# MaverickPeter/MR_SLAM

Hardware: AMD Instinct MI355X
Metric: loop-candidate pairs/sec (BEV+Radon+corr), 120k-pt scans (higher is better)
Workload: dtype f32; 1 GPU; BASELINE configs[1] batched: 120k-pt synthetic lidar scans -> Cartesian BEV 120x120x1 -> Radon 120x120 -> normalise -> half spectrum -> FFT-domain rotation correlation vs 1 candidate of the database (+ 1 query per launch swept over the database)

## Files before the change

mr_slam_amd/csrc/ringfft.hip:

```cpp
#include <algorithm>
#include <atomic>
#include <cmath>
#include <cstdlib>
#include <type_traits>

#include <hip/hip_fp16.h>

#include "common.hpp"
#include "fft_codelets.hpp"

namespace {

constexpr int kA = 120;
constexpr int kD = 120;
constexpr int kHalf = 61;
constexpr int kSlotThreads = 128;

constexpr int kLdsStride = 128;

__device__ __forceinline__ v2f cmul_conj(v2f a, v2f b)
{
    const v2f t = a.yx * b.yy * (v2f){1.0f, -1.0f};
    return __builtin_elementwise_fma(a, b.xx, t);
}

__device__ __forceinline__ v2f twiddle120(int K, v2f d)
{
    const v2f t = d.yx * (v2f){-kSin120[K], kSin120[K]};
    return __builtin_elementwise_fma(d, (v2f){kCos120[K], kCos120[K]}, t);
}

__device__ __forceinline__ void irfft_pre_pair(int J, v2f u, v2f w, v2f& zj, v2f& zp)
{
    const v2f e = __builtin_elementwise_fma(w, (v2f){1.0f, -1.0f}, u);
    const v2f d = __builtin_elementwise_fma(w, (v2f){-1.0f, 1.0f}, u);
    const v2f o = twiddle120(J, d);
    zj = __builtin_elementwise_fma(o.yx, (v2f){-1.0f, 1.0f}, e);
    zp = __builtin_elementwise_fma(e, (v2f){1.0f, -1.0f}, o.yx);
}

constexpr int kPairsPerGroup = 5;
template <class LoadA, class LoadB>
__device__ __forceinline__ void corr_irfft120(LoadA la, LoadB lb, v2f (&x)[60])
{
    constexpr int G = kPairsPerGroup, NG = 30 / kPairsPerGroup;
    v2f abuf[2][2 * G + 1];
    auto request = [&](int g, v2f (&dst)[2 * G + 1]) {
#pragma unroll
        for (int j = 0; j < G; ++j) {
            dst[2 * j] = la(g * G + j);
            dst[2 * j + 1] = la(60 - (g * G + j));
        }
        if (g == NG - 1) dst[2 * G] = la(30);
    };
    request(0, abuf[0]);
#pragma unroll
    for (int g = 0; g < NG; ++g) {
        if (g + 1 < NG) request(g + 1, abuf[(g + 1) & 1]);
        __builtin_amdgcn_sched_barrier(0);
        const v2f(&a)[2 * G + 1] = abuf[g & 1];
#pragma unroll
        for (int j = 0; j < G; ++j) {
            const int J = g * G + j;
            v2f zj, zp;
            irfft_pre_pair(J, cmul_conj(a[2 * j], lb(J)), cmul_conj(a[2 * j + 1], lb(60 - J)), zj, zp);
            x[J] = zj;
            if (J != 0) x[60 - J] = zp;
        }
        if (g == NG - 1) {
            const v2f pm = cmul_conj(a[2 * G], lb(30));
            v2f unused;
            irfft_pre_pair(30, pm, pm, x[30], unused);
        }
    }
    cfft60_inv(x);
}

__device__ __forceinline__ void rfft_post_pair(int K, v2f zk, v2f zp, v2f& xk, v2f& xp)
{
    const v2f sum = __builtin_elementwise_fma(zp, (v2f){1.0f, -1.0f}, zk);
    const v2f d = __builtin_elementwise_fma(zp, (v2f){-1.0f, 1.0f}, zk);
    const v2f tt = d.yx * (v2f){kSin120[K], -kSin120[K]};
    const v2f t = __builtin_elementwise_fma(d, (v2f){kCos120[K], kCos120[K]}, tt);
    xk = __builtin_elementwise_fma(t.yx, (v2f){1.0f, -1.0f}, sum);
    xp = __builtin_elementwise_fma(sum, (v2f){1.0f, -1.0f}, -t.yx);
}

template <class Store>
__device__ __forceinline__ void rfft120(v2f (&x)[60], Store store)
{
    cfft60_fwd(x);
#pragma unroll
    for (int K = 0; K <= 30; ++K) {
        v2f xk, xp;
        rfft_post_pair(K, x[K], x[(60 - K) % 60], xk, xp);
        store(K, xk);
        if (K != 30) store(60 - K, xp);
    }
}

constexpr float kOrtho120 = 0.09128709291752769f;

__global__ __launch_bounds__(kSlotThreads) void k_ring_half_spectrum(const float* __restrict__ x, float2* __restrict__ out,
                                                                     __half2* __restrict__ out16)
{
    const int d = min((int)threadIdx.x, kD - 1);
    const float* src = x + (size_t)blockIdx.x * kA * kD + d;
    v2f s[60];
#pragma unroll
    for (int m = 0; m < 60; ++m) s[m] = (v2f){src[(2 * m) * kD], src[(2 * m + 1) * kD]};
    const bool live = threadIdx.x < kD;
    const size_t o = (size_t)blockIdx.x * kHalf * kD + d;
    rfft120(s, [&](int k, v2f twice) {
        if (!live) return;
        const v2f v = twice * (v2f){0.5f * kOrtho120, 0.5f * kOrtho120};
        if (out) out[o + k * kD] = make_float2(v.x, v.y);
        if (out16) out16[o + k * kD] = __floats2half2_rn(v.x, v.y);
    });
}

__device__ __forceinline__ float swap32_abs_add(float a, float b)
{
    const auto r = __builtin_amdgcn_permlane32_swap(__float_as_uint(a), __float_as_uint(b), false, false);
    return fabsf(__uint_as_float(r[0])) + fabsf(__uint_as_float(r[1]));
}
__device__ __forceinline__ float swap16_add(float a, float b)
{
    const auto r = __builtin_amdgcn_permlane16_swap(__float_as_uint(a), __float_as_uint(b), false, false);
    return __uint_as_float(r[0]) + __uint_as_float(r[1]);
}

__device__ __forceinline__ void wave_abs_reduce_scatter(const v2f (&x)[60], float& w0, float& w1)
{
    const int lane = threadIdx.x & 63;
    float w[64];
#pragma unroll
    for (int i = 0; i < 64; ++i) {
        const int j = 64 + i;
        const float lo_v = (i & 1) ? x[i >> 1].y : x[i >> 1].x;
        const float hi_v = j < 120 ? ((j & 1) ? x[j >> 1].y : x[j >> 1].x) : 0.0f;
        w[i] = swap32_abs_add(lo_v, hi_v);
    }
#pragma unroll
    for (int i = 0; i < 32; ++i) w[i] = swap16_add(w[i], w[32 + i]);
#pragma unroll
    for (int step = 2; step < 6; ++step) {
        const int keep = 64 >> step;
        const int mask = 32 >> step;
        const bool hi = (lane & mask) != 0;
#pragma unroll
        for (int i = 0; i < keep; ++i) {
            const float send = hi ? w[i] : w[keep + i];
            const float mine = hi ? w[keep + i] : w[i];
            w[i] = mine + __shfl_xor(send, mask, 64);
        }
    }
    w0 = w[0];
    w1 = w[1];
}

struct FftCorrP {
    int nq, ndb, pairwise, channels;
    float denom;
    const long long* db_first;
    const long long* q_row;
    float2* mc_partial;
    int units;
};

__device__ __forceinline__ float2 load_spec(const float2* p) { return *p; }
__device__ __forceinline__ float2 load_spec(const __half2* p) { return __half22float2(*p); }

template <int NSLOT, bool QLDS, bool PAIRWISE, bool MULTI, typename DBT, bool PRELOAD = false>
__global__ __launch_bounds__(NSLOT* kSlotThreads) void k_ring_corr_fft(const float2* __restrict__ Q, const DBT* __restrict__ DB,
                                                                       FftCorrP p, float* __restrict__ dist,
                                                                       int* __restrict__ angle, float* __restrict__ corr_out)
{
    extern __shared__ __attribute__((aligned(16))) v2f qs[];
    __shared__ float xbuf[NSLOT][128];
    const int q = blockIdx.y;
    const int slot = threadIdx.x / kSlotThreads;
    const int t = threadIdx.x % kSlotThreads;
    const int wave_in_slot = t >> 6, lane = t & 63;
    const int d = min(t, kD - 1);
    const bool live_col = t < kD;
    const int C = MULTI ? p.channels : 1;
    const size_t entry = (size_t)C * kHalf * kD;
    const float2* qsrc = Q + (size_t)((!PAIRWISE && p.q_row) ? p.q_row[q] : q) * entry;
    if (!PAIRWISE && p.db_first) DB += (size_t)p.db_first[q] * entry;
    if (QLDS) {
        for (int i = threadIdx.x; i < kHalf * kLdsStride; i += NSLOT * kSlotThreads) {
            const int k = i / kLdsStride, col = i % kLdsStride;
            v2f v = {0.0f, 0.0f};
            if (col < kD) { const float2 g = qsrc[k * kD + col]; v = (v2f){g.x, g.y}; }
            qs[i] = v;
        }
        __syncthreads();
    }
    const int ncand = PAIRWISE ? 1 : p.ndb;
    const int stride = gridDim.x * NSLOT;
    const int rounds = (ncand + stride - 1) / stride;
    for (int r = 0; r < rounds; ++r) {
        const int cand = (r * gridDim.x + blockIdx.x) * NSLOT + slot;
        const bool live = cand < ncand;
        float v[2] = {0.0f, 0.0f};
        if (live) {
            for (int c = 0; c < C; ++c) {
                v2f x[60];
                const DBT* b = DB + (size_t)(PAIRWISE ? q : cand) * entry + (size_t)c * kHalf * kD + d;
                const float2* a = qsrc + (size_t)c * kHalf * kD + d;
                auto la = [&](int k) {
                    if (QLDS) return qs[k * kLdsStride + t];
                    const float2 g = a[k * kD];
                    return live_col ? (v2f){g.x, g.y} : (v2f){0.0f, 0.0f};
                };
                if (PRELOAD) {
                    DBT raw[kHalf];
#pragma unroll
                    for (int k = 0; k < kHalf; ++k) raw[k] = b[k * kD];
                    __builtin_amdgcn_sched_barrier(0);
                    corr_irfft120(la, [&](int k) { const float2 g = load_spec(&raw[k]); return (v2f){g.x, g.y}; }, x);
                } else {
                    corr_irfft120(la, [&](int k) { const float2 g = load_spec(b + k * kD); return (v2f){g.x, g.y}; }, x);
                }
                float w0, w1;
                wave_abs_reduce_scatter(x, w0, w1);
                v[0] += w0;
                v[1] += w1;
            }
        }
        if (wave_in_slot == 1) { xbuf[slot][2 * lane] = v[0]; xbuf[slot][2 * lane + 1] = v[1]; }
        __syncthreads();
        if (wave_in_slot == 0 && live) {
            const float sc = kOrtho120;
            const float s0 = (v[0] + xbuf[slot][2 * lane]) * sc, s1 = (v[1] + xbuf[slot][2 * lane + 1]) * sc;
            const int n0 = 2 * lane, n1 = 2 * lane + 1;
            const int m0 = n0 < 60 ? n0 + 60 : n0 - 60, m1 = n1 < 60 ? n1 + 60 : n1 - 60;
            const size_t o = (size_t)q * (PAIRWISE ? 1 : p.ndb) + (PAIRWISE ? 0 : cand);
            float best = -1.0f;
            int bm = 1 << 30;
            if (lane < 60) {
                if (corr_out) { corr_out[o * kA + m0] = s0; corr_out[o * kA + m1] = s1; }
                best = s0; bm = m0;
                if (s1 > best || (s1 == best && m1 < bm)) { best = s1; bm = m1; }
            }
            for (int off = 32; off > 0; off >>= 1) {
                const float ob = __shfl_xor(best, off, 64);
                const int om = __shfl_xor(bm, off, 64);
                if (ob > best || (ob == best && om < bm)) { best = ob; bm = om; }
            }
            if (lane == 0) {
                dist[o] = 1.0f - best / p.denom;
                angle[o] = kA / 2 - bm;
            }
        }
        __syncthreads();
    }
}

template <int NSLOT, typename DBT, int WAVES>
__global__ __launch_bounds__(NSLOT* kSlotThreads) __attribute__((amdgpu_waves_per_eu(WAVES, WAVES))) void k_ring_sweep_pipe(
    const float2* __restrict__ Q, const DBT* __restrict__ DB, FftCorrP p, float* __restrict__ dist, int* __restrict__ angle,
    float* __restrict__ corr_out)
{
    extern __shared__ __attribute__((aligned(16))) v2f qs[];
    __shared__ float xbuf[NSLOT][128];
    const int q = blockIdx.y;
    const int slot = threadIdx.x / kSlotThreads;
    const int t = threadIdx.x % kSlotThreads;
    const int wave_in_slot = t >> 6, lane = t & 63;
    const int d = min(t, kD - 1);
    const size_t entry = (size_t)kHalf * kD;
    const float2* qsrc = Q + (size_t)q * entry;
    const int ncand = p.ndb;
    const int stride = gridDim.x * NSLOT;
    const int rounds = (ncand + stride - 1) / stride;
    int cand = blockIdx.x * NSLOT + slot;
    DBT nxt[kHalf];
    auto fetch = [&](int c) {
        const DBT* b = DB + (size_t)c * entry + d;
#pragma unroll
        for (int k = 0; k < kHalf; ++k) nxt[k] = b[k * kD];
    };
    if (cand < ncand) fetch(cand);
    for (int i = threadIdx.x; i < kHalf * kLdsStride; i += NSLOT * kSlotThreads) {
        const int k = i / kLdsStride, col = i % kLdsStride;
        v2f v = {0.0f, 0.0f};
        if (col < kD) { const float2 g = qsrc[k * kD + col]; v = (v2f){g.x, g.y}; }
        qs[i] = v;
    }
    __syncthreads();
    for (int r = 0; r < rounds; ++r) {
        const bool live = cand < ncand;
        DBT cur[kHalf];
#pragma unroll
        for (int k = 0; k < kHalf; ++k) cur[k] = nxt[k];
        const int next = cand + stride;
        if (next < ncand) fetch(next);
        __builtin_amdgcn_sched_barrier(0);
        float v0 = 0.0f, v1 = 0.0f;
        if (live) {
            v2f x[60];
            corr_irfft120([&](int k) { return qs[k * kLdsStride + t]; },
                          [&](int k) { const float2 g = load_spec(&cur[k]); return (v2f){g.x, g.y}; }, x);
            wave_abs_reduce_scatter(x, v0, v1);
        }
        if (wave_in_slot == 1) { xbuf[slot][2 * lane] = v0; xbuf[slot][2 * lane + 1] = v1; }
        __syncthreads();
        if (wave_in_slot == 0 && live) {
            const float sc = kOrtho120;
            const float s0 = (v0 + xbuf[slot][2 * lane]) * sc, s1 = (v1 + xbuf[slot][2 * lane + 1]) * sc;
            const int n0 = 2 * lane, n1 = 2 * lane + 1;
            const int m0 = n0 < 60 ? n0 + 60 : n0 - 60, m1 = n1 < 60 ? n1 + 60 : n1 - 60;
            const size_t o = (size_t)q * p.ndb + cand;
            float best = -1.0f;
            int bm = 1 << 30;
            if (lane < 60) {
                if (corr_out) { corr_out[o * kA + m0] = s0; corr_out[o * kA + m1] = s1; }
                best = s0; bm = m0;
                if (s1 > best || (s1 == best && m1 < bm)) { best = s1; bm = m1; }
            }
            for (int off = 32; off > 0; off >>= 1) {
                const float ob = __shfl_xor(best, off, 64);
                const int om = __shfl_xor(bm, off, 64);
                if (ob > best || (ob == best && om < bm)) { best = ob; bm = om; }
            }
            if (lane == 0) {
                dist[o] = 1.0f - best / p.denom;
                angle[o] = kA / 2 - bm;
            }
        }
        __syncthreads();
        cand = next;
    }
}

constexpr int kRing = 8;
constexpr int kElems = 32;
constexpr int kSlotBytes = 1024;
constexpr int kTiledHalf1 = 30 * 1024 + 512;
constexpr int kTiledEntryBytes = 58624;
constexpr int kTiledEntry = kTiledEntryBytes / 8;


#define MRS_GLDS(MOD) asm volatile("s_mov_b32 %0, m0\n\ts_mov_b32 m0, %3\n\ts_nop 0\n\tglobal_load_lds_dwordx4 %1, %2" MOD "\n\ts_mov_b32 m0, %0" \
                                   : "=&s"(keep) : "v"(voff), "s"(sbase), "s"(lds_dst) : "memory")
template <bool NT>
__device__ __forceinline__ void glds16(const void* sbase, unsigned voff, unsigned lds_dst)
{
    unsigned keep;
    if (NT) MRS_GLDS(" nt");
    else MRS_GLDS("");
}
#undef MRS_GLDS

template <int N>
__device__ __forceinline__ void wait_vmcnt()
{
    asm volatile("s_waitcnt vmcnt(%0)" ::"n"(N) : "memory");
}

__device__ __forceinline__ void wave_abs_reduce_scatter_masked(const v2f (&x)[60], float m, float& w0, float& w1)
{
    const int lane = threadIdx.x & 63;
    float w[64];
#pragma unroll
    for (int i = 0; i < 64; ++i) {
        const int j = 64 + i;
        const float lo_v = (i & 1) ? x[i >> 1].y : x[i >> 1].x;
        const float hi_v = j < 120 ? ((j & 1) ? x[j >> 1].y : x[j >> 1].x) : 0.0f;
        const auto r = __builtin_amdgcn_permlane32_swap(__float_as_uint(lo_v), __float_as_uint(hi_v), false, false);
        w[i] = __builtin_fmaf(fabsf(__uint_as_float(r[1])), m, fabsf(__uint_as_float(r[0])));
    }
#pragma unroll
    for (int i = 0; i < 32; ++i) w[i] = swap16_add(w[i], w[32 + i]);
#pragma unroll
    for (int step = 2; step < 6; ++step) {
        const int keep = 64 >> step;
        const int mask = 32 >> step;
        const bool hi = (lane & mask) != 0;
#pragma unroll
        for (int i = 0; i < keep; ++i) {
            const float send = hi ? w[i] : w[keep + i];
            const float mine = hi ? w[keep + i] : w[i];
            w[i] = mine + __shfl_xor(send, mask, 64);
        }
    }
    w0 = w[0];
    w1 = w[1];
}

__device__ __forceinline__ void sweep_epilogue(float s0, float s1, int lane, float denom, float* dist_o, int* angle_o)
{
    const int n0 = 2 * lane, n1 = 2 * lane + 1;
    const int m0 = n0 < 60 ? n0 + 60 : n0 - 60, m1 = n1 < 60 ? n1 + 60 : n1 - 60;
    float best = -1.0f;
    int bm = 1 << 30;
    if (lane < 60) {
        best = s0; bm = m0;
        if (s1 > best || (s1 == best && m1 < bm)) { best = s1; bm = m1; }
    }
    for (int off = 32; off > 0; off >>= 1) {
        const float ob = __shfl_xor(best, off, 64);
        const int om = __shfl_xor(bm, off, 64);
        if (ob > best || (ob == best && om < bm)) { best = ob; bm = om; }
    }
    if (lane == 0) {
        *dist_o = 1.0f - best / denom;
        *angle_o = kA / 2 - bm;
    }
}

struct DmaUnit {
    const float2* base;
    int half;
    bool live;
};

template <int WAVES, bool NT, bool TILED, bool MC>
__global__ __launch_bounds__(WAVES * 64) void k_ring_sweep_dma(const float2* __restrict__ Q, const float2* __restrict__ DB, FftCorrP p,
                                                               float* __restrict__ dist, int* __restrict__ angle)
{
    extern __shared__ __attribute__((aligned(1024))) unsigned char smem[];
    v2f* const qs = reinterpret_cast<v2f*>(smem + WAVES * kRing * kSlotBytes);
    constexpr int kQueryVals = kHalf * kD + 8;
    const int wave = __builtin_amdgcn_readfirstlane(threadIdx.x >> 6);
    const int lane = threadIdx.x & 63;
    const unsigned lds0 = (unsigned)(size_t)(__attribute__((address_space(3))) unsigned char*)smem;
    const unsigned ring_lds = lds0 + wave * (kRing * kSlotBytes);
    const v2f* const ring = reinterpret_cast<const v2f*>(smem + wave * (kRing * kSlotBytes)) + lane;

    const size_t plane = TILED ? (size_t)kTiledEntry : (size_t)kHalf * kD;
    const size_t entry = (MC ? (size_t)p.channels : (size_t)1) * plane;
    const size_t qentry = (size_t)kHalf * kD;
    const int ncand = p.ndb;
    const bool multi = p.units > 0;
    const int bx = multi ? (int)((blockIdx.x >> 3) / p.nq) * 8 + (int)(blockIdx.x & 7) : (int)blockIdx.x;
    const int nbx = multi ? p.units : (int)gridDim.x;
    const int qy = multi ? (int)((blockIdx.x >> 3) % p.nq) : (int)blockIdx.y;
    if (multi && bx >= nbx) return;
    const int C = MC ? p.channels : 1;
    const int ch = MC ? bx % C : 0;
    const int slice = MC ? bx / C : bx;
    const int nslices = MC ? (nbx - ch + C - 1) / C : nbx;
    const int c0 = slice * WAVES + wave;
    const int cstride = nslices * WAVES;
    unsigned* const ticket = reinterpret_cast<unsigned*>(qs + kQueryVals);
    auto cand_of = [&](unsigned t) { return slice * WAVES + (int)(t % WAVES) + (int)(t / WAVES) * cstride; };

    const int piece = lane & 31;
    const bool upper = lane >= 32;
    const unsigned voff_h0 = TILED ? (unsigned)lane * 16u : (upper ? 60u * 960u : 0u) + (unsigned)piece * 16u;
    const unsigned voff_h1 = TILED ? (unsigned)kTiledHalf1 + (upper ? 448u : 0u) + (unsigned)min(piece, 27) * 16u
                                   : (upper ? 60u * 960u : 0u) + 512u + (unsigned)min(piece, 27) * 16u;
    const int vdelta = upper ? -960 : 960;
    unsigned run = 0;
    auto start_unit = [&](const DmaUnit& u) {
        run = u.half ? voff_h1 : voff_h0;
        asm volatile("" : "+v"(run));
    };
    auto issue = [&](const DmaUnit& u, int e) {
        if (e == 0) start_unit(u);
        const unsigned voff = (!u.live || e == kElems - 1) ? 0u : run;
        glds16<NT>(u.base, voff, ring_lds + (e % kRing) * kSlotBytes);
        if (TILED) run += u.half ? 896u : 1024u;
        else run += (unsigned)vdelta;
    };
    auto unit_of = [&](int c, int h) {
        DmaUnit u;
        u.live = c < ncand;
        u.base = DB + (size_t)(u.live ? c : 0) * entry + (size_t)ch * plane;
        u.half = h;
        return u;
    };

    const float2* const qsrc = Q + ((size_t)qy * C + (size_t)ch) * qentry;
    {
        constexpr int kPieces = (kHalf * kD * 8 + kSlotBytes - 1) / kSlotBytes;
        const unsigned q_lds = lds0 + WAVES * (kRing * kSlotBytes);
        if (threadIdx.x < 8) qs[kHalf * kD + threadIdx.x] = (v2f){0.0f, 0.0f};
        for (int pc = wave; pc < kPieces; pc += WAVES)
            if (pc * kSlotBytes + lane * 16 < kHalf * kD * 8) glds16<false>(qsrc, (unsigned)(pc * kSlotBytes + lane * 16), q_lds + pc * kSlotBytes);
    }
    DmaUnit cur = unit_of(c0, 0);
#pragma unroll
    for (int e = 0; e < kRing; ++e) issue(cur, e);
    wait_vmcnt<kRing>();
    if (threadIdx.x == 0) *ticket = WAVES;
    asm volatile("s_waitcnt lgkmcnt(0)\n\ts_barrier" ::: "memory");

    constexpr int PF = 2;
    int c = c0;
    float accA0 = 0.0f, accA1 = 0.0f;
    while (cur.live) {
        DmaUnit nxt;
        int c_next = c + cstride;
        if (cur.half == 0) nxt = unit_of(c, 1);
        else {
            unsigned t = 0;
            if (lane == 0) t = __hip_atomic_fetch_add(ticket, 1u, __ATOMIC_RELAXED, __HIP_MEMORY_SCOPE_WORKGROUP);
            c_next = cand_of(__builtin_amdgcn_readfirstlane(t));
            nxt = unit_of(c_next, 0);
        }
        const int h = cur.half;
        const v2f* const qcol = qs + h * 64 + lane;
        const float m = (h == 1 && piece >= 24) ? 0.0f : 1.0f;

        v2f x[60];
        v2f qa[PF + 1][2], cb[PF + 1][2];
        auto read_elem = [&](int e) {
            const int J = e;
            qa[e % (PF + 1)][0] = qcol[J * kD];
            cb[e % (PF + 1)][0] = ring[(e % kRing) * 128];
            if (e < 30) {
                qa[e % (PF + 1)][1] = qcol[(60 - J) * kD];
                cb[e % (PF + 1)][1] = ring[(e % kRing) * 128 + 64];
            }
        };
        __builtin_amdgcn_s_setprio(1);
        wait_vmcnt<kRing - 1>(); read_elem(0);
        wait_vmcnt<kRing - 2>(); read_elem(1);
#pragma unroll
        for (int e = 0; e < kElems; ++e) {
            if (e + PF <= 30) {
                wait_vmcnt<kRing - 1 - PF>();
                read_elem(e + PF);
            }
            if (e < 30) {
                v2f zj, zp;
                irfft_pre_pair(e, cmul_conj(qa[e % (PF + 1)][0], cb[e % (PF + 1)][0]), cmul_conj(qa[e % (PF + 1)][1], cb[e % (PF + 1)][1]), zj, zp);
                x[e] = zj;
                if (e != 0) x[60 - e] = zp;
            } else if (e == 30) {
                const v2f pm = cmul_conj(qa[e % (PF + 1)][0], cb[e % (PF + 1)][0]);
                v2f unused;
                irfft_pre_pair(30, pm, pm, x[30], unused);
            }
            __builtin_amdgcn_sched_barrier(0);
            if (e + kRing < kElems) issue(cur, e + kRing);
            else issue(nxt, e + kRing - kElems);
        }
        __builtin_amdgcn_s_setprio(0);
        cfft60_inv(x);
        float w0, w1;
        wave_abs_reduce_scatter_masked(x, m, w0, w1);

        if (MC) {
            p.mc_partial[(((size_t)qy * C + ch) * p.ndb + c) * 128 + h * 64 + lane] = make_float2(w0, w1);
            if (h == 1) c = c_next;
        } else if (h == 0) {
            accA0 = w0; accA1 = w1;
        } else {
            const float s0 = (accA0 + w0) * kOrtho120, s1 = (accA1 + w1) * kOrtho120;
            const size_t o = (size_t)qy * p.ndb + c;
            sweep_epilogue(s0, s1, lane, p.denom, dist + o, angle + o);
            c = c_next;
        }
        cur = nxt;
    }
    wait_vmcnt<0>();
}

__global__ __launch_bounds__(256) void k_ring_mc_finish(const float2* __restrict__ partial, int ndb, int C, float denom, float* __restrict__ dist,
                                                        int* __restrict__ angle)
{
    const int cand = blockIdx.x * 4 + (threadIdx.x >> 6), lane = threadIdx.x & 63;
    if (cand >= ndb) return;
    partial += (size_t)blockIdx.y * C * ndb * 128;
    float2 lo = make_float2(0.0f, 0.0f), hi = make_float2(0.0f, 0.0f);
    for (int c = 0; c < C; ++c) {
        const float2 a = partial[((size_t)c * ndb + cand) * 128 + lane], b = partial[((size_t)c * ndb + cand) * 128 + 64 + lane];
        lo.x += a.x; lo.y += a.y; hi.x += b.x; hi.y += b.y;
    }
    const size_t o = (size_t)blockIdx.y * ndb + cand;
    sweep_epilogue((lo.x + hi.x) * kOrtho120, (lo.y + hi.y) * kOrtho120, lane, denom, dist + o, angle + o);
}

__global__ __launch_bounds__(256) void k_ring_spec_to_tiled(const float2* __restrict__ src, float2* __restrict__ dst)
{
    const float2* s = src + (size_t)blockIdx.x * kHalf * kD;
    float2* d = dst + (size_t)blockIdx.x * kTiledEntry;
    for (int i = threadIdx.x; i < kTiledEntry; i += 256) {
        float2 v = make_float2(0.0f, 0.0f);
        if (i < kHalf * kD) {
            int row, col;
            if (i < kTiledHalf1 / 8) {
                const int e = i / 128, r = i % 128;
                row = r < 64 ? e : 60 - e;
                col = r % 64;
            } else {
                const int j = i - kTiledHalf1 / 8;
                const int e = j / 112, r = j % 112;
                row = r < 56 ? e : 60 - e;
                col = 64 + r % 56;
            }
            v = s[row * kD + col];
        }
        d[i] = v;
    }
}

template <int NSLOT, int MAXR, typename DBT>
__global__ __launch_bounds__(NSLOT* kSlotThreads) void k_ring_sweep_mc(const float2* __restrict__ Q, const DBT* __restrict__ DB, FftCorrP p,
                                                                       float* __restrict__ dist, int* __restrict__ angle,
                                                                       float* __restrict__ corr_out)
{
    extern __shared__ __attribute__((aligned(16))) v2f qs[];
    v2f* acc = qs + kHalf * kLdsStride;
    const int q = blockIdx.x, chunk = blockIdx.y, nchunks = gridDim.y;
    const int slot = threadIdx.x / kSlotThreads;
    const int t = threadIdx.x % kSlotThreads;
    const int lane = t & 63;
    const int d = min(t, kD - 1);
    const int C = p.channels;
    const size_t plane = (size_t)kHalf * kD, entry = (size_t)C * plane;
    const float2* qsrc = Q + (size_t)q * entry;
    const int ncand = p.ndb;
    const int rounds = (ncand + nchunks * NSLOT - 1) / (nchunks * NSLOT);
    for (int r = 0; r < rounds; ++r) acc[(r * NSLOT + slot) * kSlotThreads + t] = (v2f){0.0f, 0.0f};
    for (int c = 0; c < C; ++c) {
        __syncthreads();
        for (int i = threadIdx.x; i < kHalf * kLdsStride; i += NSLOT * kSlotThreads) {
            const int k = i / kLdsStride, col = i % kLdsStride;
            v2f v = {0.0f, 0.0f};
            if (col < kD) { const float2 g = qsrc[c * plane + k * kD + col]; v = (v2f){g.x, g.y}; }
            qs[i] = v;
        }
        __syncthreads();
        for (int r = 0; r < rounds; ++r) {
            const int cand = (r * nchunks + chunk) * NSLOT + slot;
            if (cand >= ncand) continue;
            const DBT* b = DB + (size_t)cand * entry + c * plane + d;
            DBT raw[kHalf];
#pragma unroll
            for (int k = 0; k < kHalf; ++k) raw[k] = b[k * kD];
            __builtin_amdgcn_sched_barrier(0);
            v2f x[60];
            corr_irfft120([&](int k) { return qs[k * kLdsStride + t]; },
                          [&](int k) { const float2 g = load_spec(&raw[k]); return (v2f){g.x, g.y}; }, x);
            float w0, w1;
            wave_abs_reduce_scatter(x, w0, w1);
            v2f* a = &acc[(r * NSLOT + slot) * kSlotThreads + t];
            const v2f old = *a;
            *a = (v2f){old.x + w0, old.y + w1};
        }
    }
    __syncthreads();
    if (t >= 64) return;
    for (int r = 0; r < rounds; ++r) {
        const int cand = (r * nchunks + chunk) * NSLOT + slot;
        if (cand >= ncand) continue;
        const v2f lo = acc[(r * NSLOT + slot) * kSlotThreads + lane], hi = acc[(r * NSLOT + slot) * kSlotThreads + 64 + lane];
        const float sc = kOrtho120;
        const float s0 = (lo.x + hi.x) * sc, s1 = (lo.y + hi.y) * sc;
        const int n0 = 2 * lane, n1 = 2 * lane + 1;
        const int m0 = n0 < 60 ? n0 + 60 : n0 - 60, m1 = n1 < 60 ? n1 + 60 : n1 - 60;
        const size_t o = (size_t)q * p.ndb + cand;
        float best = -1.0f;
        int bm = 1 << 30;
        if (lane < 60) {
            if (corr_out) { corr_out[o * kA + m0] = s0; corr_out[o * kA + m1] = s1; }
            best = s0; bm = m0;
            if (s1 > best || (s1 == best && m1 < bm)) { best = s1; bm = m1; }
        }
        for (int off = 32; off > 0; off >>= 1) {
            const float ob = __shfl_xor(best, off, 64);
            const int om = __shfl_xor(bm, off, 64);
            if (ob > best || (ob == best && om < bm)) { best = ob; bm = om; }
        }
        if (lane == 0) {
            dist[o] = 1.0f - best / p.denom;
            angle[o] = kA / 2 - bm;
        }
    }
}

template <typename CT>
__global__ __launch_bounds__(kSlotThreads) __attribute__((amdgpu_waves_per_eu(1, 1))) void k_ring_spec_corr_pairs(const float* __restrict__ x, const CT* __restrict__ cand,
                                                                       const int* __restrict__ cand_idx, int n_db,
                                                                       float2* __restrict__ out, __half2* __restrict__ out16,
                                                                       float denom, float* __restrict__ dist,
                                                                       int* __restrict__ angle)
{
    extern __shared__ __attribute__((aligned(16))) v2f qs[];
    __shared__ float xbuf[128];
    const int pair = blockIdx.x;
    const int t = threadIdx.x, wave = t >> 6, lane = t & 63;
    const int d = min(t, kD - 1);
    const bool live_col = t < kD;
    const int row = cand_idx ? cand_idx[pair] : pair;
    const bool no_row = cand_idx && (row < 0 || row >= n_db);
    CT raw[kHalf];
    {
        const CT* b = cand + (size_t)(no_row ? 0 : row) * kHalf * kD + d;
#pragma unroll
        for (int k = 0; k < kHalf; ++k) raw[k] = b[k * kD];
    }
    {
        const float* src = x + (size_t)pair * kA * kD + d;
        v2f s[60];
#pragma unroll
        for (int m = 0; m < 60; ++m) s[m] = (v2f){src[(2 * m) * kD], src[(2 * m + 1) * kD]};
        const size_t o = (size_t)pair * kHalf * kD + d;
        rfft120(s, [&](int k, v2f twice) {
            const v2f v = twice * (v2f){0.5f * kOrtho120, 0.5f * kOrtho120};
            qs[k * kLdsStride + t] = live_col ? v : (v2f){0.0f, 0.0f};
            if (!live_col) return;
            if (out) out[o + k * kD] = make_float2(v.x, v.y);
            if (out16) out16[o + k * kD] = __floats2half2_rn(v.x, v.y);
        });
    }
    __syncthreads();
    if (no_row) {
        if (t == 0) { dist[pair] = INFINITY; angle[pair] = 0; }
        return;
    }
    v2f c[60];
    corr_irfft120([&](int k) { return qs[k * kLdsStride + t]; },
                  [&](int k) { const float2 g = load_spec(&raw[k]); return (v2f){g.x, g.y}; }, c);
    float v0, v1;
    wave_abs_reduce_scatter(c, v0, v1);
    if (wave == 1) { xbuf[2 * lane] = v0; xbuf[2 * lane + 1] = v1; }
    __syncthreads();
    if (wave == 0) {
        const float sc = kOrtho120;
        const float s0 = (v0 + xbuf[2 * lane]) * sc, s1 = (v1 + xbuf[2 * lane + 1]) * sc;
        const int n0 = 2 * lane, n1 = 2 * lane + 1;
        const int m0 = n0 < 60 ? n0 + 60 : n0 - 60, m1 = n1 < 60 ? n1 + 60 : n1 - 60;
        float best = -1.0f;
        int bm = 1 << 30;
        if (lane < 60) {
            best = s0; bm = m0;
            if (s1 > best || (s1 == best && m1 < bm)) { best = s1; bm = m1; }
        }
        for (int off = 32; off > 0; off >>= 1) {
            const float ob = __shfl_xor(best, off, 64);
            const int om = __shfl_xor(bm, off, 64);
            if (ob > best || (ob == best && om < bm)) { best = ob; bm = om; }
        }
        if (lane == 0) {
            dist[pair] = 1.0f - best / denom;
            angle[pair] = kA / 2 - bm;
        }
    }
}

}

template <typename CT>
static int spectrum_corr_pairs_launch(mrs_ctx* ctx, const float* d_norm_sino, const CT* cand, const int32_t* d_cand_index,
                                      int32_t n_db, int32_t n_pairs, int32_t n_angles, int32_t det, float* d_half_spec, void* d_half_spec_f16,
                                      float* d_dist, int32_t* d_angle, mrs_stream stream)
{
    MRS_REQUIRE(ctx && d_norm_sino && cand && d_dist && d_angle, "null pointer");
    MRS_REQUIRE(n_pairs > 0, "n_pairs must be positive");
    if (n_angles != kA || det != kD) {
        mrs::set_error("ring_spectrum_corr_pairs is specialised for 120 x 120 (got %d x %d)", n_angles, det);
        return MRS_ERR_UNSUPPORTED;
    }
    MRS_HIP_TRY(hipSetDevice(ctx->device));
    const size_t lds = (size_t)kHalf * kLdsStride * sizeof(v2f);
    MRS_HIP_TRY(hipFuncSetAttribute(reinterpret_cast<const void*>(k_ring_spec_corr_pairs<CT>), hipFuncAttributeMaxDynamicSharedMemorySize,
                                    (int)lds));
    hipLaunchKernelGGL(k_ring_spec_corr_pairs<CT>, dim3(n_pairs), dim3(kSlotThreads), lds, (hipStream_t)stream, d_norm_sino, cand,
                       d_cand_index, n_db, reinterpret_cast<float2*>(d_half_spec), reinterpret_cast<__half2*>(d_half_spec_f16),
                       (float)(0.15 * kA * kD), d_dist, d_angle);
    MRS_HIP_TRY(hipGetLastError());
    return MRS_OK;
}

extern "C" {

static int half_spectrum_launch(mrs_ctx* ctx, const float* d_norm_sino, int32_t n_img, int32_t n_angles, int32_t det,
                                float* d_half_spec, void* d_half_spec_f16, mrs_stream stream)
{
    MRS_REQUIRE(ctx && d_norm_sino && (d_half_spec || d_half_spec_f16), "null pointer");
    MRS_REQUIRE(n_img > 0, "n_img must be positive");
    if (n_angles != kA || det != kD) {
        mrs::set_error("ring_half_spectrum is specialised for 120 x 120 (got %d x %d)", n_angles, det);
        return MRS_ERR_UNSUPPORTED;
    }
    MRS_HIP_TRY(hipSetDevice(ctx->device));
    hipLaunchKernelGGL(k_ring_half_spectrum, dim3(n_img), dim3(kSlotThreads), 0, (hipStream_t)stream, d_norm_sino,
                       reinterpret_cast<float2*>(d_half_spec), reinterpret_cast<__half2*>(d_half_spec_f16));
    MRS_HIP_TRY(hipGetLastError());
    return MRS_OK;
}

int mrs_ring_half_spectrum(mrs_ctx* ctx, const float* d_norm_sino, int32_t n_img, int32_t n_angles, int32_t det,
                           float* d_half_spec, mrs_stream stream)
{
    MRS_REQUIRE(d_half_spec, "null pointer");
    return half_spectrum_launch(ctx, d_norm_sino, n_img, n_angles, det, d_half_spec, nullptr, stream);
}

int mrs_ring_half_spectrum_f16(mrs_ctx* ctx, const float* d_norm_sino, int32_t n_img, int32_t n_angles, int32_t det,
                               float* d_half_spec, void* d_half_spec_f16, mrs_stream stream)
{
    return half_spectrum_launch(ctx, d_norm_sino, n_img, n_angles, det, d_half_spec, d_half_spec_f16, stream);
}

extern "C++" {
template <int WAVES, bool NT, bool TILED, bool MC>
static hipError_t sweep_dma_launch_t(int num_cu, hipStream_t s, const float2* q, const float2* db, const FftCorrP& p, float* dist, int* angle)
{
    const size_t lds = (size_t)WAVES * kRing * kSlotBytes + (size_t)(kHalf * kD + 8) * sizeof(v2f) + 16 ;
    auto kern = k_ring_sweep_dma<WAVES, NT, TILED, MC>;
    static std::atomic<unsigned> attr_set{0};
    int dev = 0;
    hipError_t e = hipGetDevice(&dev);
    if (e != hipSuccess) return e;
    if (!(attr_set.load(std::memory_order_relaxed) & (1u << (dev & 31)))) {
        e = hipFuncSetAttribute(reinterpret_cast<const void*>(kern), hipFuncAttributeMaxDynamicSharedMemorySize, (int)lds);
        if (e != hipSuccess) return e;
        attr_set.fetch_or(1u << (dev & 31), std::memory_order_relaxed);
    }
    const int C = MC ? p.channels : 1;
    const int need = C * ((p.ndb + WAVES - 1) / WAVES);
    if (p.nq > 1) {
        FftCorrP pm = p;
        pm.units = std::max(C, std::min(std::max(8, num_cu / (8 * p.nq) * 8), need));
        const int grid = (pm.units + 7) / 8 * 8 * p.nq;
        hipLaunchKernelGGL(kern, dim3(grid, 1), dim3(WAVES * 64), lds, s, q, db, pm, dist, angle);
        return hipGetLastError();
    }
    int blocks = std::max(1, std::min(num_cu, need));
    if (MC) blocks = std::max(p.channels, blocks);
    hipLaunchKernelGGL(kern, dim3(blocks, 1), dim3(WAVES * 64), lds, s, q, db, p, dist, angle);
    return hipGetLastError();
}
template <bool TILED, bool MC>
static hipError_t sweep_dma_launch(int num_cu, hipStream_t s, const float2* q, const float2* db, const FftCorrP& p, float* dist, int* angle)
{
    return p.nq > 1 ? sweep_dma_launch_t<12, false, TILED, MC>(num_cu, s, q, db, p, dist, angle)
                    : sweep_dma_launch_t<8, true, TILED, MC>(num_cu, s, q, db, p, dist, angle);
}

constexpr int kSweepDmaMaxQ = 32;
constexpr int kSweepDmaMaxQMc = 8;

static int sweep_dma_mc(mrs_ctx* ctx, hipStream_t s, const float2* q, const float2* db, FftCorrP p, float* dist, int* angle, bool tiled)
{
    mrs::Scratch part;
    int st = part.alloc((size_t)p.nq * p.channels * p.ndb * 128 * sizeof(float2), s);
    if (st != MRS_OK) return st;
    p.mc_partial = part.as<float2>();
    const int num_cu = ctx->num_cu > 0 ? ctx->num_cu : 256;
    if (tiled) MRS_HIP_TRY((sweep_dma_launch<true, true>(num_cu, s, q, db, p, dist, angle)));
    else MRS_HIP_TRY((sweep_dma_launch<false, true>(num_cu, s, q, db, p, dist, angle)));
    hipLaunchKernelGGL(k_ring_mc_finish, dim3((p.ndb + 3) / 4, p.nq), dim3(256), 0, s, p.mc_partial, p.ndb, p.channels, p.denom, dist, angle);
    MRS_HIP_TRY(hipGetLastError());
    return MRS_OK;
}

static int sweep_dma_queries(mrs_ctx* ctx, hipStream_t s, const float2* q, int n_q, const float2* db, FftCorrP p, float* dist, int* angle, bool tiled)
{
    const int num_cu = ctx->num_cu > 0 ? ctx->num_cu : 256;
    const int C = p.channels;
    const int maxq = C > 1 ? kSweepDmaMaxQMc : kSweepDmaMaxQ;
    const size_t qentry = (size_t)C * kHalf * kD;
    for (int q0 = 0; q0 < n_q; q0 += maxq) {
        p.nq = std::min(maxq, n_q - q0);
        const float2* qq = q + (size_t)q0 * qentry;
        float* dd = dist + (size_t)q0 * p.ndb;
        int* aa = angle + (size_t)q0 * p.ndb;
        if (C > 1) {
            const int st = sweep_dma_mc(ctx, s, qq, db, p, dd, aa, tiled);
            if (st != MRS_OK) return st;
            continue;
        }
        if (tiled) MRS_HIP_TRY((sweep_dma_launch<true, false>(num_cu, s, qq, db, p, dd, aa)));
        else MRS_HIP_TRY((sweep_dma_launch<false, false>(num_cu, s, qq, db, p, dd, aa)));
    }
    return MRS_OK;
}

template <typename DBT>
static int corr_fft_launch(mrs_ctx* ctx, const float* d_q, int32_t n_q, const void* d_db, int32_t n_db, int32_t channels,
                           float* d_dist, int32_t* d_angle, float* d_corr, mrs_stream stream, bool pairwise,
                           const long long* d_db_first = nullptr, const long long* d_q_row = nullptr)
{
    MRS_REQUIRE(ctx && d_q && d_db && d_dist && d_angle, "null pointer");
    MRS_REQUIRE(n_q > 0 && n_db > 0 && channels > 0, "counts must be positive");
    MRS_HIP_TRY(hipSetDevice(ctx->device));
    FftCorrP p;
    p.nq = n_q; p.ndb = n_db; p.pairwise = pairwise ? 1 : 0; p.channels = channels;
    p.denom = (float)(0.15 * channels * kA * kD);
    p.db_first = d_db_first; p.q_row = d_q_row; p.mc_partial = nullptr; p.units = 0;
    MRS_REQUIRE(!(d_db_first || d_q_row) || (!pairwise && channels == 1 && std::is_same<DBT, float2>::value && n_q <= mrs::kMaxGridY),
                "per-query database blocks: single-channel fp32 sweeps of at most 65535 queries");
    constexpr int NSLOT = 2;
    hipStream_t s = (hipStream_t)stream;
    const float2* q2 = reinterpret_cast<const float2*>(d_q);
    const DBT* db2 = reinterpret_cast<const DBT*>(d_db);
    const size_t entry = (size_t)channels * kHalf * kD;
    for (int q0 = 0; q0 < n_q; q0 += mrs::kMaxGridY) {
        const int nq = std::min(n_q - q0, mrs::kMaxGridY);
        p.nq = nq;
        const size_t ro = (size_t)q0 * (pairwise ? 1 : n_db);
        const float2* qq = q2 + q0 * entry;
        const DBT* dd = pairwise ? db2 + q0 * entry : db2;
        float* dist_c = d_dist + ro;
        int32_t* angle_c = d_angle + ro;
        float* corr_c = d_corr ? d_corr + ro * kA : nullptr;
        if (pairwise) {
            if (channels == 1)
                hipLaunchKernelGGL((k_ring_corr_fft<1, false, true, false, DBT>), dim3(1, nq), dim3(kSlotThreads), 0, s, qq, dd, p, dist_c,
                                   angle_c, corr_c);
            else
                hipLaunchKernelGGL((k_ring_corr_fft<1, false, true, true, DBT>), dim3(1, nq), dim3(kSlotThreads), 0, s, qq, dd, p, dist_c,
                                   angle_c, corr_c);
        } else {
            int blocks = 2 * (ctx->num_cu > 0 ? ctx->num_cu : 256);
            if (n_q > 1) blocks = (blocks + n_q - 1) / n_q;
            const int need = (n_db + NSLOT - 1) / NSLOT;
            if (blocks > need) blocks = need;
            if (blocks < 1) blocks = 1;
            if (channels == 1) {
                const size_t lds = (size_t)kHalf * kLdsStride * sizeof(v2f);
                bool launched = false;
                if constexpr (std::is_same<DBT, float2>::value) {
                    if (nq <= kSweepDmaMaxQ && !d_corr && !d_db_first && !d_q_row) {
                        const int st = sweep_dma_queries(ctx, s, qq, nq, dd, p, dist_c, angle_c, false);
                        if (st != MRS_OK) return st;
                        launched = true;
                    }
                }
                if constexpr (std::is_same<DBT, __half2>::value) {
                    if (n_q <= 2) {
                        auto kern = k_ring_sweep_pipe<NSLOT, DBT, 2>;
                        MRS_HIP_TRY(hipFuncSetAttribute(reinterpret_cast<const void*>(kern), hipFuncAttributeMaxDynamicSharedMemorySize, (int)lds));
                        hipLaunchKernelGGL(kern, dim3(blocks, nq), dim3(NSLOT * kSlotThreads), lds, s, qq, dd, p, dist_c, angle_c, corr_c);
                        launched = true;
                    }
                }
                if (!launched) {
                    auto kern = k_ring_corr_fft<NSLOT, true, false, false, DBT, true>;
                    MRS_HIP_TRY(hipFuncSetAttribute(reinterpret_cast<const void*>(kern), hipFuncAttributeMaxDynamicSharedMemorySize, (int)lds));
                    hipLaunchKernelGGL(kern, dim3(blocks, nq), dim3(NSLOT * kSlotThreads), lds, s, qq, dd, p, dist_c, angle_c, corr_c);
                }
            } else if (std::is_same<DBT, float2>::value && nq <= kSweepDmaMaxQMc && !d_corr) {
                const int st = sweep_dma_queries(ctx, s, qq, nq, reinterpret_cast<const float2*>(dd), p, dist_c, angle_c, false);
                if (st != MRS_OK) return st;
            } else {
                constexpr int MAXR = 8;
                const int resident = std::max(1, 2 * (ctx->num_cu > 0 ? ctx->num_cu : 256) / nq);
                const int waves = (n_db + NSLOT * MAXR * resident - 1) / (NSLOT * MAXR * resident);
                const int chunks = std::max(1, std::min(waves * resident, (n_db + NSLOT - 1) / NSLOT));
                const size_t lds = (size_t)(kHalf * kLdsStride + MAXR * NSLOT * kSlotThreads) * sizeof(v2f);
                if (chunks <= mrs::kMaxGridY) {
                    auto kern = k_ring_sweep_mc<NSLOT, MAXR, DBT>;
                    MRS_HIP_TRY(hipFuncSetAttribute(reinterpret_cast<const void*>(kern), hipFuncAttributeMaxDynamicSharedMemorySize, (int)lds));
                    hipLaunchKernelGGL(kern, dim3(nq, chunks), dim3(NSLOT * kSlotThreads), lds, s, qq, dd, p, dist_c, angle_c, corr_c);
                } else {
                    hipLaunchKernelGGL((k_ring_corr_fft<NSLOT, false, false, true, DBT>), dim3(blocks, nq), dim3(NSLOT * kSlotThreads), 0, s, qq, dd,
                                       p, dist_c, angle_c, corr_c);
                }
            }
        }
    }
    MRS_HIP_TRY(hipGetLastError());
    return MRS_OK;
}
}

int mrs_ring_corr_fft_sweep(mrs_ctx* ctx, const float* d_query_spec, int32_t n_query, const float* d_db_spec,
                            int32_t n_db, float* d_dist, int32_t* d_angle, float* d_corr, mrs_stream stream)
{
    return corr_fft_launch<float2>(ctx, d_query_spec, n_query, d_db_spec, n_db, 1, d_dist, d_angle, d_corr, stream, false);
}

int mrs_ring_spec_to_tiled(mrs_ctx* ctx, const float* d_half_spec, int32_t n, float* d_tiled, mrs_stream stream)
{
    MRS_REQUIRE(ctx && d_half_spec && d_tiled, "null pointer");
    MRS_REQUIRE(n > 0, "n must be positive");
    MRS_HIP_TRY(hipSetDevice(ctx->device));
    hipLaunchKernelGGL(k_ring_spec_to_tiled, dim3(n), dim3(256), 0, (hipStream_t)stream, reinterpret_cast<const float2*>(d_half_spec),
                       reinterpret_cast<float2*>(d_tiled));
    MRS_HIP_TRY(hipGetLastError());
    return MRS_OK;
}

int mrs_ring_corr_fft_sweep_tiled_q(mrs_ctx* ctx, const float* d_query_spec, int32_t n_query, const float* d_db_tiled, int32_t n_db, int32_t channels,
                                    float* d_dist, int32_t* d_angle, mrs_stream stream)
{
    MRS_REQUIRE(ctx && d_query_spec && d_db_tiled && d_dist && d_angle, "null pointer");
    MRS_REQUIRE(n_query > 0 && n_db > 0 && channels > 0, "counts must be positive");
    MRS_HIP_TRY(hipSetDevice(ctx->device));
    FftCorrP p;
    p.nq = 1; p.ndb = n_db; p.pairwise = 0; p.channels = channels;
    p.denom = (float)(0.15 * channels * kA * kD);
    p.db_first = nullptr; p.q_row = nullptr; p.mc_partial = nullptr; p.units = 0;
    return sweep_dma_queries(ctx, (hipStream_t)stream, reinterpret_cast<const float2*>(d_query_spec), n_query, reinterpret_cast<const float2*>(d_db_tiled), p,
                             d_dist, d_angle, true);
}

int mrs_ring_corr_fft_sweep_tiled(mrs_ctx* ctx, const float* d_query_spec, const float* d_db_tiled, int32_t n_db, int32_t channels, float* d_dist,
                                  int32_t* d_angle, mrs_stream stream)
{
    return mrs_ring_corr_fft_sweep_tiled_q(ctx, d_query_spec, 1, d_db_tiled, n_db, channels, d_dist, d_angle, stream);
}

int mrs_ring_corr_fft_sweep_blocks(mrs_ctx* ctx, const float* d_spec, const int64_t* d_query_row, int32_t n_query, const int64_t* d_db_first,
                                   int32_t n_db, float* d_dist, int32_t* d_angle, mrs_stream stream)
{
    MRS_REQUIRE(d_query_row && d_db_first, "null pointer");
    static_assert(sizeof(long long) == sizeof(int64_t), "int64_t is long long here");
    return corr_fft_launch<float2>(ctx, d_spec, n_query, d_spec, n_db, 1, d_dist, d_angle, nullptr, stream, false,
                                   reinterpret_cast<const long long*>(d_db_first), reinterpret_cast<const long long*>(d_query_row));
}

int mrs_ring_corr_fft_sweep_f16(mrs_ctx* ctx, const float* d_query_spec, int32_t n_query, const void* d_db_spec_f16,
                                int32_t n_db, float* d_dist, int32_t* d_angle, float* d_corr, mrs_stream stream)
{
    return corr_fft_launch<__half2>(ctx, d_query_spec, n_query, d_db_spec_f16, n_db, 1, d_dist, d_angle, d_corr, stream, false);
}

int mrs_ring_corr_fft_pairs(mrs_ctx* ctx, const float* d_a_spec, const float* d_b_spec, int32_t n_pairs, float* d_dist,
                            int32_t* d_angle, float* d_corr, mrs_stream stream)
{
    return corr_fft_launch<float2>(ctx, d_a_spec, n_pairs, d_b_spec, n_pairs, 1, d_dist, d_angle, d_corr, stream, true);
}

int mrs_ring_corr_fft_sweep_mc(mrs_ctx* ctx, const float* d_query_spec, int32_t n_query, const float* d_db_spec, int32_t n_db,
                               int32_t channels, float* d_dist, int32_t* d_angle, float* d_corr, mrs_stream stream)
{
    return corr_fft_launch<float2>(ctx, d_query_spec, n_query, d_db_spec, n_db, channels, d_dist, d_angle, d_corr, stream, false);
}

int mrs_ring_corr_fft_pairs_mc(mrs_ctx* ctx, const float* d_a_spec, const float* d_b_spec, int32_t n_pairs, int32_t channels,
                               float* d_dist, int32_t* d_angle, float* d_corr, mrs_stream stream)
{
    return corr_fft_launch<float2>(ctx, d_a_spec, n_pairs, d_b_spec, n_pairs, channels, d_dist, d_angle, d_corr, stream, true);
}

int mrs_ring_spectrum_corr_pairs(mrs_ctx* ctx, const float* d_norm_sino, const float* d_cand_spec, int32_t n_pairs,
                                 int32_t n_angles, int32_t det, float* d_half_spec, void* d_half_spec_f16, float* d_dist,
                                 int32_t* d_angle, mrs_stream stream)
{
    return spectrum_corr_pairs_launch<float2>(ctx, d_norm_sino, reinterpret_cast<const float2*>(d_cand_spec), nullptr, n_pairs, n_pairs, n_angles,
                                              det, d_half_spec, d_half_spec_f16, d_dist, d_angle, stream);
}

int mrs_ring_spectrum_corr_pairs_db(mrs_ctx* ctx, const float* d_norm_sino, const void* d_db_spec, int32_t db_is_f16, int32_t n_db,
                                    const int32_t* d_cand_index, int32_t n_pairs, int32_t n_angles, int32_t det, float* d_half_spec,
                                    void* d_half_spec_f16, float* d_dist, int32_t* d_angle, mrs_stream stream)
{
    MRS_REQUIRE(d_cand_index, "null candidate index");
    MRS_REQUIRE(n_db > 0, "n_db must be positive");
    return db_is_f16 ? spectrum_corr_pairs_launch<__half2>(ctx, d_norm_sino, reinterpret_cast<const __half2*>(d_db_spec), d_cand_index,
                                                          n_db, n_pairs, n_angles, det, d_half_spec, d_half_spec_f16, d_dist, d_angle, stream)
                     : spectrum_corr_pairs_launch<float2>(ctx, d_norm_sino, reinterpret_cast<const float2*>(d_db_spec), d_cand_index,
                                                          n_db, n_pairs, n_angles, det, d_half_spec, d_half_spec_f16, d_dist, d_angle, stream);
}

}
```

Measured before the change: 2.436 million pairs/s.

## Make spectrum-correlation kernel persistent with register-prefetched sinograms and fused products

Turns the per-pair correlation kernel into a grid-strided persistent kernel sized to twice the CU count. Each block prefetches the next pair's sinogram into registers, split across the inverse FFT, to hide global load latency. The conjugate product is fused into the forward FFT's store callback, which removes the LDS staging of the query spectrum and one barrier. The optional half-spectrum outputs become compile-time template variants. In exchange register pressure rises sharply (raw, prod, s and c arrays all live at once), which risks spills, and parallelism is capped at a fixed grid.

```diff
diff --git a/mr_slam_amd/csrc/ringfft.hip b/mr_slam_amd/csrc/ringfft.hip
--- a/mr_slam_amd/csrc/ringfft.hip
+++ b/mr_slam_amd/csrc/ringfft.hip
@@ -73,6 +73,23 @@
             irfft_pre_pair(30, pm, pm, x[30], unused);
         }
     }
+    cfft60_inv(x);
+}
+
+template <class Prod, class Mid>
+__device__ __forceinline__ void irfft120_products(Prod p, v2f (&x)[60], Mid mid)
+{
+#pragma unroll
+    for (int J = 0; J < 30; ++J) {
+        v2f zj, zp;
+        irfft_pre_pair(J, p(J), p(60 - J), zj, zp);
+        x[J] = zj;
+        if (J != 0) x[60 - J] = zp;
+    }
+    const v2f pm = p(30);
+    v2f unused;
+    irfft_pre_pair(30, pm, pm, x[30], unused);
+    mid();
     cfft60_inv(x);
 }
 
@@ -675,73 +692,96 @@
     }
 }
 
-template <typename CT>
+template <typename CT, int OUT>
 __global__ __launch_bounds__(kSlotThreads) __attribute__((amdgpu_waves_per_eu(1, 1))) void k_ring_spec_corr_pairs(const float* __restrict__ x, const CT* __restrict__ cand,
-                                                                       const int* __restrict__ cand_idx, int n_db,
+                                                                       const int* __restrict__ cand_idx, int n_db, int n_pairs,
                                                                        float2* __restrict__ out, __half2* __restrict__ out16,
                                                                        float denom, float* __restrict__ dist,
                                                                        int* __restrict__ angle)
 {
-    extern __shared__ __attribute__((aligned(16))) v2f qs[];
-    __shared__ float xbuf[128];
-    const int pair = blockIdx.x;
+    __shared__ float xbuf[2][128];
     const int t = threadIdx.x, wave = t >> 6, lane = t & 63;
     const int d = min(t, kD - 1);
     const bool live_col = t < kD;
-    const int row = cand_idx ? cand_idx[pair] : pair;
-    const bool no_row = cand_idx && (row < 0 || row >= n_db);
-    CT raw[kHalf];
-    {
-        const CT* b = cand + (size_t)(no_row ? 0 : row) * kHalf * kD + d;
-#pragma unroll
-        for (int k = 0; k < kHalf; ++k) raw[k] = b[k * kD];
-    }
-    {
-        const float* src = x + (size_t)pair * kA * kD + d;
-        v2f s[60];
-#pragma unroll
-        for (int m = 0; m < 60; ++m) s[m] = (v2f){src[(2 * m) * kD], src[(2 * m + 1) * kD]};
-        const size_t o = (size_t)pair * kHalf * kD + d;
-        rfft120(s, [&](int k, v2f twice) {
-            const v2f v = twice * (v2f){0.5f * kOrtho120, 0.5f * kOrtho120};
-            qs[k * kLdsStride + t] = live_col ? v : (v2f){0.0f, 0.0f};
-            if (!live_col) return;
-            if (out) out[o + k * kD] = make_float2(v.x, v.y);
-            if (out16) out16[o + k * kD] = __floats2half2_rn(v.x, v.y);
-        });
-    }
-    __syncthreads();
-    if (no_row) {
-        if (t == 0) { dist[pair] = INFINITY; angle[pair] = 0; }
-        return;
-    }
-    v2f c[60];
-    corr_irfft120([&](int k) { return qs[k * kLdsStride + t]; },
-                  [&](int k) { const float2 g = load_spec(&raw[k]); return (v2f){g.x, g.y}; }, c);
-    float v0, v1;
-    wave_abs_reduce_scatter(c, v0, v1);
-    if (wave == 1) { xbuf[2 * lane] = v0; xbuf[2 * lane + 1] = v1; }
-    __syncthreads();
-    if (wave == 0) {
-        const float sc = kOrtho120;
-        const float s0 = (v0 + xbuf[2 * lane]) * sc, s1 = (v1 + xbuf[2 * lane + 1]) * sc;
-        const int n0 = 2 * lane, n1 = 2 * lane + 1;
-        const int m0 = n0 < 60 ? n0 + 60 : n0 - 60, m1 = n1 < 60 ? n1 + 60 : n1 - 60;
-        float best = -1.0f;
-        int bm = 1 << 30;
-        if (lane < 60) {
-            best = s0; bm = m0;
-            if (s1 > best || (s1 == best && m1 < bm)) { best = s1; bm = m1; }
-        }
-        for (int off = 32; off > 0; off >>= 1) {
-            const float ob = __shfl_xor(best, off, 64);
-            const int om = __shfl_xor(bm, off, 64);
-            if (ob > best || (ob == best && om < bm)) { best = ob; bm = om; }
-        }
-        if (lane == 0) {
-            dist[pair] = 1.0f - best / denom;
-            angle[pair] = kA / 2 - bm;
-        }
+    const int stride = gridDim.x;
+    int pair = blockIdx.x;
+    int row = cand_idx ? cand_idx[pair] : pair;
+    int par = 0;
+    v2f s[60];
+    auto request_sino = [&](int p, int m0, int m1) {
+        const float* src = x + (size_t)p * kA * kD + d;
+#pragma unroll
+        for (int m = m0; m < m1; ++m) s[m] = (v2f){src[(2 * m) * kD], src[(2 * m + 1) * kD]};
+        __builtin_amdgcn_sched_barrier(0);
+    };
+    request_sino(pair, 0, 60);
+    for (;;) {
+        const int next = pair + stride;
+        const bool more = next < n_pairs;
+        const int row_next = more && cand_idx ? cand_idx[next] : next;
+        const bool no_row = cand_idx && (row < 0 || row >= n_db);
+        CT raw[kHalf];
+        {
+            const CT* b = cand + (size_t)(no_row ? 0 : row) * kHalf * kD + d;
+#pragma unroll
+            for (int k = 0; k < kHalf; ++k) raw[k] = b[k * kD];
+            __builtin_amdgcn_sched_barrier(0);
+        }
+        v2f prod[kHalf];
+        {
+            const size_t o = (size_t)pair * kHalf * kD + d;
+            rfft120(s, [&](int k, v2f twice) {
+                const v2f v = twice * (v2f){0.5f * kOrtho120, 0.5f * kOrtho120};
+                const float2 g = load_spec(&raw[k]);
+                prod[k] = cmul_conj(live_col ? v : (v2f){0.0f, 0.0f}, (v2f){g.x, g.y});
+                if (!live_col) return;
+                if (OUT & 1) out[o + k * kD] = make_float2(v.x, v.y);
+                if (OUT & 2) out16[o + k * kD] = __floats2half2_rn(v.x, v.y);
+            });
+        }
+        __builtin_amdgcn_sched_barrier(0);
+        const int ahead = more ? next : pair;
+        request_sino(ahead, 0, 30);
+        auto mid = [&] {
+            __builtin_amdgcn_sched_barrier(0);
+            request_sino(ahead, 30, 60);
+        };
+        if (!no_row) {
+            v2f c[60];
+            irfft120_products([&](int k) { return prod[k]; }, c, mid);
+            float v0, v1;
+            wave_abs_reduce_scatter(c, v0, v1);
+            if (wave == 1) { xbuf[par][2 * lane] = v0; xbuf[par][2 * lane + 1] = v1; }
+            __syncthreads();
+            if (wave == 0) {
+                const float sc = kOrtho120;
+                const float s0 = (v0 + xbuf[par][2 * lane]) * sc, s1 = (v1 + xbuf[par][2 * lane + 1]) * sc;
+                const int n0 = 2 * lane, n1 = 2 * lane + 1;
+                const int m0 = n0 < 60 ? n0 + 60 : n0 - 60, m1 = n1 < 60 ? n1 + 60 : n1 - 60;
+                float best = -1.0f;
+                int bm = 1 << 30;
+                if (lane < 60) {
+                    best = s0; bm = m0;
+                    if (s1 > best || (s1 == best && m1 < bm)) { best = s1; bm = m1; }
+                }
+                for (int off = 32; off > 0; off >>= 1) {
+                    const float ob = __shfl_xor(best, off, 64);
+                    const int om = __shfl_xor(bm, off, 64);
+                    if (ob > best || (ob == best && om < bm)) { best = ob; bm = om; }
+                }
+                if (lane == 0) {
+                    dist[pair] = 1.0f - best / denom;
+                    angle[pair] = kA / 2 - bm;
+                }
+            }
+            par ^= 1;
+        } else {
+            if (t == 0) { dist[pair] = INFINITY; angle[pair] = 0; }
+            mid();
+        }
+        if (!more) break;
+        pair = next;
+        row = row_next;
     }
 }
 
@@ -759,12 +799,18 @@
         return MRS_ERR_UNSUPPORTED;
     }
     MRS_HIP_TRY(hipSetDevice(ctx->device));
-    const size_t lds = (size_t)kHalf * kLdsStride * sizeof(v2f);
-    MRS_HIP_TRY(hipFuncSetAttribute(reinterpret_cast<const void*>(k_ring_spec_corr_pairs<CT>), hipFuncAttributeMaxDynamicSharedMemorySize,
-                                    (int)lds));
-    hipLaunchKernelGGL(k_ring_spec_corr_pairs<CT>, dim3(n_pairs), dim3(kSlotThreads), lds, (hipStream_t)stream, d_norm_sino, cand,
-                       d_cand_index, n_db, reinterpret_cast<float2*>(d_half_spec), reinterpret_cast<__half2*>(d_half_spec_f16),
-                       (float)(0.15 * kA * kD), d_dist, d_angle);
+    const int grid = std::min<int>(n_pairs, 2 * (ctx->num_cu > 0 ? ctx->num_cu : 256));
+    auto launch = [&](auto which) {
+        hipLaunchKernelGGL((k_ring_spec_corr_pairs<CT, decltype(which)::value>), dim3(grid), dim3(kSlotThreads), 0, (hipStream_t)stream,
+                           d_norm_sino, cand, d_cand_index, n_db, n_pairs, reinterpret_cast<float2*>(d_half_spec),
+                           reinterpret_cast<__half2*>(d_half_spec_f16), (float)(0.15 * kA * kD), d_dist, d_angle);
+    };
+    switch ((d_half_spec ? 1 : 0) | (d_half_spec_f16 ? 2 : 0)) {
+        case 0: launch(std::integral_constant<int, 0>{}); break;
+        case 1: launch(std::integral_constant<int, 1>{}); break;
+        case 2: launch(std::integral_constant<int, 2>{}); break;
+        default: launch(std::integral_constant<int, 3>{}); break;
+    }
     MRS_HIP_TRY(hipGetLastError());
     return MRS_OK;
 }
```

Measured after the change: 2.497 million pairs/s (median of 6 runs). +2.5%, better.
